# vinits5/learning3d

Hardware: AMD Instinct MI355X
Metric: clouds/sec DGCNN-fwd+Chamfer B=32 N=1024; kNN HBM GB/s vs peak at 1/2/4/8 GPU (higher is better)
Workload: dtype f32 (shared-MLP GEMMs as f16x2: fp32 operands carried as an fp16 high part + an fp16 residual (unscaled between the EdgeConv kernel and conv5, 2^12-scaled elsewhere), 3 fp16 MFMA products per fp32 product, f32 accumulate, fp32-level error -- tests bound it by 2x the fp32-MFMA kernel's own error agai

## Files before the change

### learning3d_amd/csrc/knn_mfma.hip

```cpp
#include "common.h"

typedef float f32x16 __attribute__((ext_vector_type(16)));
typedef unsigned long long u64;

#define KM_MCAP 64
#define KM_STRIDE 65
#define KM_WPAD 16
#define KM_T3S 25
#define KM_PAD (-3.0e38f)

__device__ __forceinline__ f32x16 km_tile(const float *__restrict__ cxy, const float *__restrict__ czw, int at,
                                          float b1, float b2, float b3, float a3)
{
    f32x16 acc = {0.f, 0.f, 0.f, 0.f, 0.f, 0.f, 0.f, 0.f, 0.f, 0.f, 0.f, 0.f, 0.f, 0.f, 0.f, 0.f};
    acc = __builtin_amdgcn_mfma_f32_32x32x2f32(cxy[at], b1, acc, 0, 0, 0);
    acc = __builtin_amdgcn_mfma_f32_32x32x2f32(czw[at], b2, acc, 0, 0, 0);
    acc = __builtin_amdgcn_mfma_f32_32x32x2f32(a3, b3, acc, 0, 0, 0);
    return acc;
}

__device__ __forceinline__ float km_nextup(float x)
{
    const unsigned b = __float_as_uint(x + 0.0f);
    return __uint_as_float((int)b >= 0 ? b + 1u : b - 1u);
}

#ifdef KM_TIMING
#define KMT(n) if (lane == 0) ((long long *)idx_out)[((size_t)(blockIdx.y * gridDim.x + blockIdx.x) * 4 + wave) * 16 + (n)] = __builtin_amdgcn_s_memtime();
#else
#define KMT(n)
#endif

template <int CT>
__global__ __launch_bounds__(256, 2) void knn_mfma_kernel(const float *__restrict__ xyz, int N, int k, int T_,
                                                          int64_t *__restrict__ idx_out)
{
    const int T = CT > 0 ? CT : T_;
    extern __shared__ __attribute__((aligned(16))) unsigned char km_smem[];
    const int NS = 4 * T * 32, WS = T * 32 + KM_WPAD, P = 4 * WS;
    float *cx = (float *)km_smem;
    float *cz = cx + 2 * P;
    float *dump = cx + 4 * P;
    u64 *qlist = (u64 *)(dump + 4 * 2048);
    float *t3 = (float *)(qlist + 32 * KM_STRIDE);
    float *thr0s = t3 + 32 * KM_T3S;
    int *qcnt = (int *)(thr0s + 32 * 9);
    int *ovf = qcnt + 32;

    const int tid = threadIdx.x, lane = tid & 63, wave = tid >> 6;
    const int i = lane & 31, h = lane >> 5, lane8 = 2 * wave + h;
    const int b = blockIdx.y, q0 = blockIdx.x * 32;
    const float *cloud = xyz + (size_t)b * N * 3;
    KMT(7)

    for (int c0 = tid; c0 < NS; c0 += 1024) {
        float x[4], y[4], z[4];
#pragma unroll
        for (int u = 0; u < 4; u++) {
            const int cc = min(c0 + 256 * u, N - 1);
            x[u] = cloud[cc * 3 + 0];
            y[u] = cloud[cc * 3 + 1];
            z[u] = cloud[cc * 3 + 2];
        }
#pragma unroll
        for (int u = 0; u < 4; u++)
            if (c0 + 256 * u >= N) { x[u] = 0.f; y[u] = 0.f; z[u] = 0.f; }
#pragma unroll
        for (int u = 0; u < 4; u++) {
            const int c = c0 + 256 * u;
            if (c < NS) {
                const float w = c < N ? -((x[u] * x[u] + y[u] * y[u]) + z[u] * z[u]) : KM_PAD;
                const int l8 = c & 7, s = c >> 3, j = s >> 4, r = s & 15;
                const int p = (l8 >> 1) * WS + j * 32 + ((r >> 2) << 3) + ((l8 & 1) << 2) + (r & 3);
                cx[p] = x[u];
                cx[P + p] = y[u];
                cz[p] = z[u];
                cz[P + p] = w;
            }
        }
    }
    for (int e = tid; e < 32 * KM_STRIDE; e += 256) qlist[e] = 0ull;
    if (tid < 32) qcnt[tid] = 0;
    if (tid == 0) *ovf = 0;

    const int q = q0 + i;
    const bool valid = q < N;
    const float *qp = cloud + (size_t)(valid ? q : N - 1) * 3;
    const float qx = qp[0], qy = qp[1], qz = qp[2];
    const float qxx = (qx * qx + qy * qy) + qz * qz;
    const float b1 = h ? 2.0f * qy : 2.0f * qx;
    const float b2 = h ? 1.0f : 2.0f * qz;
    const float b3 = h ? 0.0f : -qxx;
    const float a3 = h ? 0.0f : 1.0f;
    const float *cxy = cx + h * P;
    const float *czw = cz + h * P;
    const int at0 = wave * WS + i;
    KMT(0)
    __syncthreads();
    KMT(1)

    float mr[16];
#pragma unroll
    for (int r = 0; r < 16; r++) mr[r] = -INFINITY;
    f32x16 kept[CT > 0 ? CT : 1];
    int j = 0;
    if constexpr (CT > 0) {
        static_assert(CT % 2 == 0, "tiles are consumed in pairs");
#pragma unroll
        for (int t = 0; t < CT; t++) kept[t] = km_tile(cxy, czw, at0 + t * 32, b1, b2, b3, a3);
#pragma unroll
        for (int t = 0; t < CT; t += 2)
#pragma unroll
            for (int r = 0; r < 16; r++) mr[r] = fmaxf(fmaxf(mr[r], kept[t][r]), kept[t + 1][r]);
    } else {
        for (; j + 2 <= T; j += 2) {
            const f32x16 aA = km_tile(cxy, czw, at0 + j * 32, b1, b2, b3, a3);
            const f32x16 aB = km_tile(cxy, czw, at0 + j * 32 + 32, b1, b2, b3, a3);
#pragma unroll
            for (int r = 0; r < 16; r++) mr[r] = fmaxf(fmaxf(mr[r], aA[r]), aB[r]);
        }
        if (j < T) {
            const f32x16 aA = km_tile(cxy, czw, at0 + j * 32, b1, b2, b3, a3);
#pragma unroll
            for (int r = 0; r < 16; r++) mr[r] = fmaxf(mr[r], aA[r]);
        }
    }
    KMT(2)
    float m1 = -INFINITY, m2 = -INFINITY, m3 = -INFINITY;
#pragma unroll
    for (int r = 0; r < 16; r++) {
        const float v = mr[r];
        m3 = __builtin_amdgcn_fmed3f(m2, m3, v);
        m2 = __builtin_amdgcn_fmed3f(m1, m2, v);
        m1 = fmaxf(m1, v);
    }
    t3[i * KM_T3S + lane8 * 3 + 0] = m1;
    t3[i * KM_T3S + lane8 * 3 + 1] = m2;
    t3[i * KM_T3S + lane8 * 3 + 2] = m3;
    __syncthreads();
    {
        int g1 = 0, g2 = 0, g3 = 0;
#pragma unroll 8
        for (int f = 0; f < 24; f++) {
            const float v = t3[i * KM_T3S + f];
            g1 += v > m1;
            g2 += v > m2;
            g3 += v > m3;
        }
        const float offer = g3 < k ? m3 : g2 < k ? m2 : g1 < k ? m1 : INFINITY;
        thr0s[i * 9 + lane8] = offer;
    }
    __syncthreads();
    float thr0_ = thr0s[i * 9];
#pragma unroll
    for (int l = 1; l < 8; l++) thr0_ = fminf(thr0_, thr0s[i * 9 + l]);
#ifdef KM_TIMING
    float thr0 = (k & 0x100) ? INFINITY : thr0_;
    k &= 0xff;
#else
    float thr0 = thr0_;
#endif
    KMT(3)

    float *mydump = dump + wave * 2048;
    u64 *mylist = qlist + i * KM_STRIDE;
    float thr = thr0;
    bool strict = false;
    for (int attempt = 0;; attempt++) {
        const float thrc = strict ? km_nextup(thr) : thr;
        bool over = false;
    #pragma unroll
        for (j = 0; j < T; j += 2) {
            const bool two = j + 1 < T;
            f32x16 aA, aB;
            if constexpr (CT > 0) {
                aA = kept[j];
                aB = kept[j + 1];
            } else {
                aA = km_tile(cxy, czw, at0 + j * 32, b1, b2, b3, a3);
                aB = km_tile(cxy, czw, at0 + (two ? j * 32 + 32 : j * 32), b1, b2, b3, a3);
            }
            unsigned sgn = 0;
    #pragma unroll
            for (int r = 0; r < 16; r++) sgn = __builtin_amdgcn_alignbit(sgn, __float_as_uint(aA[r] - thrc), 31);
    #pragma unroll
            for (int r = 0; r < 16; r++) sgn = __builtin_amdgcn_alignbit(sgn, __float_as_uint(aB[r] - thrc), 31);
            unsigned m = ~sgn;
            if (!two) m &= 0xFFFF0000u;
            if (__builtin_amdgcn_ballot_w64(m != 0) != 0) {
    #pragma unroll
                for (int qd = 0; qd < 4; qd++) {
                    *(float4 *)(mydump + (qd * 64 + lane) * 4) = make_float4(aA[4 * qd], aA[4 * qd + 1], aA[4 * qd + 2], aA[4 * qd + 3]);
                    *(float4 *)(mydump + 1024 + (qd * 64 + lane) * 4) = make_float4(aB[4 * qd], aB[4 * qd + 1], aB[4 * qd + 2], aB[4 * qd + 3]);
                }
                const int cbase = 128 * j + lane8;
    #pragma unroll 1
                do {
                    int e[4], slot[4];
                    bool has[4];
                    float vv[4];
    #pragma unroll
                    for (int u = 0; u < 4; u++) {
                        has[u] = m != 0;
                        e[u] = has[u] ? __builtin_clz(m) : 31;
                        m &= ~(0x80000000u >> e[u]);
                        vv[u] = mydump[((e[u] >> 2) << 8) + lane * 4 + (e[u] & 3)];
                        slot[u] = atomicAdd(&qcnt[i], has[u] ? 1 : 0);
                    }
    #pragma unroll
                    for (int u = 0; u < 4; u++) {
                        const unsigned bits = __float_as_uint(vv[u] + 0.0f);
                        const unsigned sk = bits ^ ((unsigned)((int)bits >> 31) | 0x80000000u);
                        const u64 key = ((u64)sk << 32) | (unsigned)(~(cbase + 8 * e[u]));
                        const bool fits = slot[u] < KM_MCAP;
                        over |= has[u] && !fits;
                        mylist[has[u] && fits ? slot[u] : KM_MCAP] = key;
                    }
                } while (__builtin_amdgcn_ballot_w64(m != 0) != 0);
            }
        }
        if (over) *ovf = 1;
        KMT(4)
        __syncthreads();
        KMT(5)
        if (*ovf == 0) break;
        if (attempt == 64) {
            if (tid == 0) idx_out[((size_t)b * N + q0) * k] = -1;
            return;
        }
        if (lane8 == 0) thr0s[i * 9 + 8] = thr;
        __syncthreads();
        {
            u64 own[8];
            int rank[8];
#pragma unroll
            for (int o = 0; o < 8; o++) {
                own[o] = mylist[lane8 + 8 * o];
                rank[o] = 0;
            }
            for (int f = 0; f < KM_MCAP; f++) {
                const u64 kf = mylist[f];
#pragma unroll
                for (int o = 0; o < 8; o++) rank[o] += kf > own[o] ? 1 : 0;
            }
#pragma unroll
            for (int o = 0; o < 8; o++)
                if (own[o] != 0ull && rank[o] == k - 1) {
                    const unsigned sk = (unsigned)(own[o] >> 32);
                    thr0s[i * 9 + 8] = __uint_as_float((sk & 0x80000000u) ? sk ^ 0x80000000u : ~sk);
                }
        }
        __syncthreads();
        {
            const float thr_new = thr0s[i * 9 + 8];
            if (thr_new > thr) {
                thr = thr_new;
                strict = false;
            } else {
                strict = true;
            }
        }
        __syncthreads();
        for (int e = tid; e < 32 * KM_STRIDE; e += 256) qlist[e] = 0ull;
        if (tid < 32) qcnt[tid] = 0;
        if (tid == 0) *ovf = 0;
        __syncthreads();
    }

    int Mi = qcnt[i];
#pragma unroll
    for (int d = 16; d > 0; d >>= 1) Mi = max(Mi, __shfl_xor(Mi, d, 64));
    const int Mmax = __builtin_amdgcn_readfirstlane(Mi);
    u64 own[8];
    int rank[8];
#pragma unroll
    for (int o = 0; o < 8; o++) {
        own[o] = mylist[lane8 + 8 * o];
        rank[o] = 0;
    }
    if (Mmax <= 32) {
#pragma unroll 2
        for (int f = 0; f < Mmax; f++) {
            const u64 kf = mylist[f];
#pragma unroll
            for (int o = 0; o < 4; o++) rank[o] += kf > own[o] ? 1 : 0;
        }
    } else if (Mmax <= 48) {
#pragma unroll 2
        for (int f = 0; f < Mmax; f++) {
            const u64 kf = mylist[f];
#pragma unroll
            for (int o = 0; o < 6; o++) rank[o] += kf > own[o] ? 1 : 0;
        }
    } else {
#pragma unroll 2
        for (int f = 0; f < Mmax; f++) {
            const u64 kf = mylist[f];
#pragma unroll
            for (int o = 0; o < 8; o++) rank[o] += kf > own[o] ? 1 : 0;
        }
    }
    KMT(6)
#ifdef KM_TIMING
    if (lane == 0) ((long long *)idx_out)[((size_t)(blockIdx.y * gridDim.x + blockIdx.x) * 4 + wave) * 16 + 8] =
        rank[0] + rank[1] + rank[2] + rank[3] + rank[4] + rank[5] + rank[6] + rank[7];
    return;
#endif
    int64_t *dst = idx_out + ((size_t)b * N + (valid ? q : 0)) * k;
    if (valid) {
#pragma unroll
        for (int o = 0; o < 8; o++)
            if (own[o] != 0ull && rank[o] < k) dst[rank[o]] = (int64_t)(unsigned)(~(unsigned)own[o]);
    }

    const int Mq = qcnt[i];
    const int need = (strict && Mq < k) ? k - Mq : 0;
    __syncthreads();
    if (tid == 0) *ovf = 0;
    __syncthreads();
    if (need > 0) atomicMax(ovf, need);
    __syncthreads();
    const int rounds = *ovf;
    int last = -1;
    int *props = (int *)thr0s;
    for (int round = 0; round < rounds; round++) {
        int prop = 0x7fffffff;
        for (int t = T - 1; t >= 0; t--) {
            f32x16 av;
            if constexpr (CT > 0) {
                av = kept[0];
#pragma unroll
                for (int u = 1; u < CT; u++) av = t == u ? kept[u] : av;
            } else {
                av = km_tile(cxy, czw, at0 + t * 32, b1, b2, b3, a3);
            }
#pragma unroll
            for (int r = 15; r >= 0; r--) {
                const int sl = 16 * t + r;
                prop = (av[r] == thr && sl > last) ? sl : prop;
            }
        }
        const int c = prop != 0x7fffffff ? 8 * prop + lane8 : 0x7fffffff;
        props[i * 9 + lane8] = c;
        __syncthreads();
        int cmin = props[i * 9];
#pragma unroll
        for (int l = 1; l < 8; l++) cmin = min(cmin, props[i * 9 + l]);
        if (c == cmin && c != 0x7fffffff) {
            last = prop;
            if (round < need && valid) dst[Mq + round] = c;
        }
        __syncthreads();
    }
}

size_t l3d_knn_mfma_lds_bytes(int N)
{
    const int T = l3d_divup(N, 128);
    return (size_t)4 * (4 * (T * 32 + KM_WPAD)) * 4 + 4 * 2048 * 4 + 32 * KM_STRIDE * 8 + 32 * KM_T3S * 4 + 32 * 9 * 4 + 32 * 4 + 16;
}

bool l3d_knn_mfma_supported(int N, int k) { return k <= 24 && N >= 256 && N <= 2048; }

int l3d_launch_knn_mfma(const float *xyz, int B, int N, int k, int64_t *idx, hipStream_t st)
{
    const int T = l3d_divup(N, 128);
    const dim3 grid(l3d_divup(N, 32), B);
    if (T == 8)
        hipLaunchKernelGGL(knn_mfma_kernel<8>, grid, dim3(256), l3d_knn_mfma_lds_bytes(N), st, xyz, N, k, T, idx);
    else
        hipLaunchKernelGGL(knn_mfma_kernel<0>, grid, dim3(256), l3d_knn_mfma_lds_bytes(N), st, xyz, N, k, T, idx);
    return l3d_check_launch();
}
```

Measured before the change: 120,300.

## Double kNN block to 64 queries, drop kept tiles and LDS dump, recompute distances

The kNN kernel now uses 512-thread blocks that handle 64 queries with 8 waves, sharing one staged candidate set in LDS. The register-resident kept[] tiles and the per-wave LDS dump buffer are removed. Each pass recomputes tiles with a 2-MFMA product that leaves out the -|q|^2 term and subtracts it afterward, and selected candidates get their exact value recomputed from LDS coordinates with fmaf. The aim is to cut register and LDS pressure so occupancy rises and candidate loading is amortised, at the cost of redoing the MFMAs on every threshold attempt and possibly shifting tie-breaking numerics.

Result: faster. 122,800 (median of 6 runs) (+2.1%).

```diff
diff --git a/learning3d_amd/csrc/knn_mfma.hip b/learning3d_amd/csrc/knn_mfma.hip
--- a/learning3d_amd/csrc/knn_mfma.hip
+++ b/learning3d_amd/csrc/knn_mfma.hip
@@ -19,6 +19,20 @@
     return acc;
 }
 
+__device__ __forceinline__ f32x16 km_tile2(const float *__restrict__ cxy, const float *__restrict__ czw, int at, float b1, float b2)
+{
+    f32x16 acc = {0.f, 0.f, 0.f, 0.f, 0.f, 0.f, 0.f, 0.f, 0.f, 0.f, 0.f, 0.f, 0.f, 0.f, 0.f, 0.f};
+    acc = __builtin_amdgcn_mfma_f32_32x32x2f32(cxy[at], b1, acc, 0, 0, 0);
+    acc = __builtin_amdgcn_mfma_f32_32x32x2f32(czw[at], b2, acc, 0, 0, 0);
+    return acc;
+}
+
+__device__ __forceinline__ float km_value(float cx, float cy, float cz, float cw, float tqx, float tqy, float tqz, float qxx)
+{
+    const float d = fmaf(cz, tqz, fmaf(cy, tqy, cx * tqx));
+    return (d + cw) - qxx;
+}
+
 __device__ __forceinline__ float km_nextup(float x)
 {
     const unsigned b = __float_as_uint(x + 0.0f);
@@ -26,13 +40,13 @@
 }
 
 #ifdef KM_TIMING
-#define KMT(n) if (lane == 0) ((long long *)idx_out)[((size_t)(blockIdx.y * gridDim.x + blockIdx.x) * 4 + wave) * 16 + (n)] = __builtin_amdgcn_s_memtime();
+#define KMT(n) if (lane == 0) ((long long *)idx_out)[((size_t)(blockIdx.y * gridDim.x + blockIdx.x) * 8 + wave) * 16 + (n)] = __builtin_amdgcn_s_memtime();
 #else
 #define KMT(n)
 #endif
 
 template <int CT>
-__global__ __launch_bounds__(256, 2) void knn_mfma_kernel(const float *__restrict__ xyz, int N, int k, int T_,
+__global__ __launch_bounds__(512, 4) void knn_mfma_kernel(const float *__restrict__ xyz, int N, int k, int T_,
                                                           int64_t *__restrict__ idx_out)
 {
     const int T = CT > 0 ? CT : T_;
@@ -40,34 +54,34 @@
     const int NS = 4 * T * 32, WS = T * 32 + KM_WPAD, P = 4 * WS;
     float *cx = (float *)km_smem;
     float *cz = cx + 2 * P;
-    float *dump = cx + 4 * P;
-    u64 *qlist = (u64 *)(dump + 4 * 2048);
-    float *t3 = (float *)(qlist + 32 * KM_STRIDE);
-    float *thr0s = t3 + 32 * KM_T3S;
-    int *qcnt = (int *)(thr0s + 32 * 9);
-    int *ovf = qcnt + 32;
-
-    const int tid = threadIdx.x, lane = tid & 63, wave = tid >> 6;
-    const int i = lane & 31, h = lane >> 5, lane8 = 2 * wave + h;
-    const int b = blockIdx.y, q0 = blockIdx.x * 32;
+    u64 *qlist = (u64 *)(cx + 4 * P);
+    float *t3 = (float *)(qlist + 64 * KM_STRIDE);
+    float *thr0s = t3 + 64 * KM_T3S;
+    int *qcnt = (int *)(thr0s + 64 * 9);
+    int *ovf = qcnt + 64;
+
+    const int tid = threadIdx.x, lane = tid & 63, wave = tid >> 6, wq = wave & 3;
+    const int i = lane & 31, h = lane >> 5, lane8 = 2 * wq + h;
+    const int qi = (wave >> 2) * 32 + i;
+    const int b = blockIdx.y, q0 = blockIdx.x * 64;
     const float *cloud = xyz + (size_t)b * N * 3;
     KMT(7)
 
-    for (int c0 = tid; c0 < NS; c0 += 1024) {
+    for (int c0 = tid; c0 < NS; c0 += 2048) {
         float x[4], y[4], z[4];
 #pragma unroll
         for (int u = 0; u < 4; u++) {
-            const int cc = min(c0 + 256 * u, N - 1);
+            const int cc = min(c0 + 512 * u, N - 1);
             x[u] = cloud[cc * 3 + 0];
             y[u] = cloud[cc * 3 + 1];
             z[u] = cloud[cc * 3 + 2];
         }
 #pragma unroll
         for (int u = 0; u < 4; u++)
-            if (c0 + 256 * u >= N) { x[u] = 0.f; y[u] = 0.f; z[u] = 0.f; }
+            if (c0 + 512 * u >= N) { x[u] = 0.f; y[u] = 0.f; z[u] = 0.f; }
 #pragma unroll
         for (int u = 0; u < 4; u++) {
-            const int c = c0 + 256 * u;
+            const int c = c0 + 512 * u;
             if (c < NS) {
                 const float w = c < N ? -((x[u] * x[u] + y[u] * y[u]) + z[u] * z[u]) : KM_PAD;
                 const int l8 = c & 7, s = c >> 3, j = s >> 4, r = s & 15;
@@ -79,22 +93,23 @@
             }
         }
     }
-    for (int e = tid; e < 32 * KM_STRIDE; e += 256) qlist[e] = 0ull;
-    if (tid < 32) qcnt[tid] = 0;
+    for (int e = tid; e < 64 * KM_STRIDE; e += 512) qlist[e] = 0ull;
+    if (tid < 64) qcnt[tid] = 0;
     if (tid == 0) *ovf = 0;
 
-    const int q = q0 + i;
+    const int q = q0 + qi;
     const bool valid = q < N;
     const float *qp = cloud + (size_t)(valid ? q : N - 1) * 3;
     const float qx = qp[0], qy = qp[1], qz = qp[2];
     const float qxx = (qx * qx + qy * qy) + qz * qz;
-    const float b1 = h ? 2.0f * qy : 2.0f * qx;
-    const float b2 = h ? 1.0f : 2.0f * qz;
+    const float tqx = 2.0f * qx, tqy = 2.0f * qy, tqz = 2.0f * qz;
+    const float b1 = h ? tqy : tqx;
+    const float b2 = h ? 1.0f : tqz;
     const float b3 = h ? 0.0f : -qxx;
     const float a3 = h ? 0.0f : 1.0f;
     const float *cxy = cx + h * P;
     const float *czw = cz + h * P;
-    const int at0 = wave * WS + i;
+    const int at0 = wq * WS + i;
     KMT(0)
     __syncthreads();
     KMT(1)
@@ -102,29 +117,21 @@
     float mr[16];
 #pragma unroll
     for (int r = 0; r < 16; r++) mr[r] = -INFINITY;
-    f32x16 kept[CT > 0 ? CT : 1];
     int j = 0;
-    if constexpr (CT > 0) {
-        static_assert(CT % 2 == 0, "tiles are consumed in pairs");
-#pragma unroll
-        for (int t = 0; t < CT; t++) kept[t] = km_tile(cxy, czw, at0 + t * 32, b1, b2, b3, a3);
-#pragma unroll
-        for (int t = 0; t < CT; t += 2)
-#pragma unroll
-            for (int r = 0; r < 16; r++) mr[r] = fmaxf(fmaxf(mr[r], kept[t][r]), kept[t + 1][r]);
-    } else {
-        for (; j + 2 <= T; j += 2) {
-            const f32x16 aA = km_tile(cxy, czw, at0 + j * 32, b1, b2, b3, a3);
-            const f32x16 aB = km_tile(cxy, czw, at0 + j * 32 + 32, b1, b2, b3, a3);
-#pragma unroll
-            for (int r = 0; r < 16; r++) mr[r] = fmaxf(fmaxf(mr[r], aA[r]), aB[r]);
-        }
-        if (j < T) {
-            const f32x16 aA = km_tile(cxy, czw, at0 + j * 32, b1, b2, b3, a3);
-#pragma unroll
-            for (int r = 0; r < 16; r++) mr[r] = fmaxf(mr[r], aA[r]);
-        }
-    }
+    for (; j + 2 <= T; j += 2) {
+        const f32x16 aA = km_tile2(cxy, czw, at0 + j * 32, b1, b2);
+        const f32x16 aB = km_tile2(cxy, czw, at0 + j * 32 + 32, b1, b2);
+#pragma unroll
+        for (int r = 0; r < 16; r++) mr[r] = fmaxf(fmaxf(mr[r], aA[r]), aB[r]);
+        __builtin_amdgcn_sched_barrier(0);
+    }
+    if (j < T) {
+        const f32x16 aA = km_tile2(cxy, czw, at0 + j * 32, b1, b2);
+#pragma unroll
+        for (int r = 0; r < 16; r++) mr[r] = fmaxf(mr[r], aA[r]);
+    }
+#pragma unroll
+    for (int r = 0; r < 16; r++) mr[r] = (mr[r] - qxx) + 0.0f;
     KMT(2)
     float m1 = -INFINITY, m2 = -INFINITY, m3 = -INFINITY;
 #pragma unroll
@@ -134,26 +141,26 @@
         m2 = __builtin_amdgcn_fmed3f(m1, m2, v);
         m1 = fmaxf(m1, v);
     }
-    t3[i * KM_T3S + lane8 * 3 + 0] = m1;
-    t3[i * KM_T3S + lane8 * 3 + 1] = m2;
-    t3[i * KM_T3S + lane8 * 3 + 2] = m3;
+    t3[qi * KM_T3S + lane8 * 3 + 0] = m1;
+    t3[qi * KM_T3S + lane8 * 3 + 1] = m2;
+    t3[qi * KM_T3S + lane8 * 3 + 2] = m3;
     __syncthreads();
     {
         int g1 = 0, g2 = 0, g3 = 0;
 #pragma unroll 8
         for (int f = 0; f < 24; f++) {
-            const float v = t3[i * KM_T3S + f];
+            const float v = t3[qi * KM_T3S + f];
             g1 += v > m1;
             g2 += v > m2;
             g3 += v > m3;
         }
         const float offer = g3 < k ? m3 : g2 < k ? m2 : g1 < k ? m1 : INFINITY;
-        thr0s[i * 9 + lane8] = offer;
-    }
-    __syncthreads();
-    float thr0_ = thr0s[i * 9];
-#pragma unroll
-    for (int l = 1; l < 8; l++) thr0_ = fminf(thr0_, thr0s[i * 9 + l]);
+        thr0s[qi * 9 + lane8] = offer;
+    }
+    __syncthreads();
+    float thr0_ = thr0s[qi * 9];
+#pragma unroll
+    for (int l = 1; l < 8; l++) thr0_ = fminf(thr0_, thr0s[qi * 9 + l]);
 #ifdef KM_TIMING
     float thr0 = (k & 0x100) ? INFINITY : thr0_;
     k &= 0xff;
@@ -162,54 +169,60 @@
 #endif
     KMT(3)
 
-    float *mydump = dump + wave * 2048;
-    u64 *mylist = qlist + i * KM_STRIDE;
+    u64 *mylist = qlist + qi * KM_STRIDE;
+    const int pbase = wq * WS + 4 * h;
     float thr = thr0;
     bool strict = false;
     for (int attempt = 0;; attempt++) {
-        const float thrc = strict ? km_nextup(thr) : thr;
+        const float thrt = strict ? km_nextup(thr) : thr;
+        const float thrc = thrt == 0.0f ? -0.0f : thrt;
         bool over = false;
-    #pragma unroll
-        for (j = 0; j < T; j += 2) {
-            const bool two = j + 1 < T;
-            f32x16 aA, aB;
-            if constexpr (CT > 0) {
-                aA = kept[j];
-                aB = kept[j + 1];
-            } else {
-                aA = km_tile(cxy, czw, at0 + j * 32, b1, b2, b3, a3);
-                aB = km_tile(cxy, czw, at0 + (two ? j * 32 + 32 : j * 32), b1, b2, b3, a3);
-            }
-            unsigned sgn = 0;
-    #pragma unroll
-            for (int r = 0; r < 16; r++) sgn = __builtin_amdgcn_alignbit(sgn, __float_as_uint(aA[r] - thrc), 31);
-    #pragma unroll
-            for (int r = 0; r < 16; r++) sgn = __builtin_amdgcn_alignbit(sgn, __float_as_uint(aB[r] - thrc), 31);
-            unsigned m = ~sgn;
-            if (!two) m &= 0xFFFF0000u;
+    #pragma unroll 1
+        for (j = 0; j < T; j += 4) {
+            u64 m = 0;
+    #pragma unroll
+            for (int jp = 0; jp < 4; jp += 2) {
+                const int jj = j + jp;
+                unsigned mp = 0;
+                if (jj < T) {
+                    const bool two = jj + 1 < T;
+                    const f32x16 aA = km_tile2(cxy, czw, at0 + jj * 32, b1, b2);
+                    const f32x16 aB = km_tile2(cxy, czw, at0 + (two ? jj * 32 + 32 : jj * 32), b1, b2);
+                    unsigned sgn = 0;
+    #pragma unroll
+                    for (int r = 0; r < 16; r++) sgn = __builtin_amdgcn_alignbit(sgn, __float_as_uint((aA[r] - qxx) - thrc), 31);
+    #pragma unroll
+                    for (int r = 0; r < 16; r++) sgn = __builtin_amdgcn_alignbit(sgn, __float_as_uint((aB[r] - qxx) - thrc), 31);
+                    mp = ~sgn;
+                    if (!two) mp &= 0xFFFF0000u;
+                }
+                m = (m << 32) | mp;
+                __builtin_amdgcn_sched_barrier(0);
+            }
             if (__builtin_amdgcn_ballot_w64(m != 0) != 0) {
-    #pragma unroll
-                for (int qd = 0; qd < 4; qd++) {
-                    *(float4 *)(mydump + (qd * 64 + lane) * 4) = make_float4(aA[4 * qd], aA[4 * qd + 1], aA[4 * qd + 2], aA[4 * qd + 3]);
-                    *(float4 *)(mydump + 1024 + (qd * 64 + lane) * 4) = make_float4(aB[4 * qd], aB[4 * qd + 1], aB[4 * qd + 2], aB[4 * qd + 3]);
-                }
+                const int pj = pbase + 32 * j;
                 const int cbase = 128 * j + lane8;
     #pragma unroll 1
                 do {
                     int e[4], slot[4];
                     bool has[4];
-                    float vv[4];
+                    float vx[4], vy[4], vz[4], vw[4];
     #pragma unroll
                     for (int u = 0; u < 4; u++) {
                         has[u] = m != 0;
-                        e[u] = has[u] ? __builtin_clz(m) : 31;
-                        m &= ~(0x80000000u >> e[u]);
-                        vv[u] = mydump[((e[u] >> 2) << 8) + lane * 4 + (e[u] & 3)];
-                        slot[u] = atomicAdd(&qcnt[i], has[u] ? 1 : 0);
+                        e[u] = has[u] ? __builtin_clzll(m) : 63;
+                        m &= ~(0x8000000000000000ull >> e[u]);
+                        const int p = pj + e[u] + (e[u] & ~3);
+                        vx[u] = cx[p];
+                        vy[u] = cx[P + p];
+                        vz[u] = cz[p];
+                        vw[u] = cz[P + p];
+                        slot[u] = atomicAdd(&qcnt[qi], has[u] ? 1 : 0);
                     }
     #pragma unroll
                     for (int u = 0; u < 4; u++) {
-                        const unsigned bits = __float_as_uint(vv[u] + 0.0f);
+                        const float vv = km_value(vx[u], vy[u], vz[u], vw[u], tqx, tqy, tqz, qxx);
+                        const unsigned bits = __float_as_uint(vv + 0.0f);
                         const unsigned sk = bits ^ ((unsigned)((int)bits >> 31) | 0x80000000u);
                         const u64 key = ((u64)sk << 32) | (unsigned)(~(cbase + 8 * e[u]));
                         const bool fits = slot[u] < KM_MCAP;
@@ -228,7 +241,7 @@
             if (tid == 0) idx_out[((size_t)b * N + q0) * k] = -1;
             return;
         }
-        if (lane8 == 0) thr0s[i * 9 + 8] = thr;
+        if (lane8 == 0) thr0s[qi * 9 + 8] = thr;
         __syncthreads();
         {
             u64 own[8];
@@ -247,12 +260,12 @@
             for (int o = 0; o < 8; o++)
                 if (own[o] != 0ull && rank[o] == k - 1) {
                     const unsigned sk = (unsigned)(own[o] >> 32);
-                    thr0s[i * 9 + 8] = __uint_as_float((sk & 0x80000000u) ? sk ^ 0x80000000u : ~sk);
+                    thr0s[qi * 9 + 8] = __uint_as_float((sk & 0x80000000u) ? sk ^ 0x80000000u : ~sk);
                 }
         }
         __syncthreads();
         {
-            const float thr_new = thr0s[i * 9 + 8];
+            const float thr_new = thr0s[qi * 9 + 8];
             if (thr_new > thr) {
                 thr = thr_new;
                 strict = false;
@@ -261,13 +274,13 @@
             }
         }
         __syncthreads();
-        for (int e = tid; e < 32 * KM_STRIDE; e += 256) qlist[e] = 0ull;
-        if (tid < 32) qcnt[tid] = 0;
+        for (int e = tid; e < 64 * KM_STRIDE; e += 512) qlist[e] = 0ull;
+        if (tid < 64) qcnt[tid] = 0;
         if (tid == 0) *ovf = 0;
         __syncthreads();
     }
 
-    int Mi = qcnt[i];
+    int Mi = qcnt[qi];
 #pragma unroll
     for (int d = 16; d > 0; d >>= 1) Mi = max(Mi, __shfl_xor(Mi, d, 64));
     const int Mmax = __builtin_amdgcn_readfirstlane(Mi);
@@ -302,7 +315,7 @@
     }
     KMT(6)
 #ifdef KM_TIMING
-    if (lane == 0) ((long long *)idx_out)[((size_t)(blockIdx.y * gridDim.x + blockIdx.x) * 4 + wave) * 16 + 8] =
+    if (lane == 0) ((long long *)idx_out)[((size_t)(blockIdx.y * gridDim.x + blockIdx.x) * 8 + wave) * 16 + 8] =
         rank[0] + rank[1] + rank[2] + rank[3] + rank[4] + rank[5] + rank[6] + rank[7];
     return;
 #endif
@@ -313,7 +326,7 @@
             if (own[o] != 0ull && rank[o] < k) dst[rank[o]] = (int64_t)(unsigned)(~(unsigned)own[o]);
     }
 
-    const int Mq = qcnt[i];
+    const int Mq = qcnt[qi];
     const int need = (strict && Mq < k) ? k - Mq : 0;
     __syncthreads();
     if (tid == 0) *ovf = 0;
@@ -326,14 +339,7 @@
     for (int round = 0; round < rounds; round++) {
         int prop = 0x7fffffff;
         for (int t = T - 1; t >= 0; t--) {
-            f32x16 av;
-            if constexpr (CT > 0) {
-                av = kept[0];
-#pragma unroll
-                for (int u = 1; u < CT; u++) av = t == u ? kept[u] : av;
-            } else {
-                av = km_tile(cxy, czw, at0 + t * 32, b1, b2, b3, a3);
-            }
+            const f32x16 av = km_tile(cxy, czw, at0 + t * 32, b1, b2, b3, a3);
 #pragma unroll
             for (int r = 15; r >= 0; r--) {
                 const int sl = 16 * t + r;
@@ -341,11 +347,11 @@
             }
         }
         const int c = prop != 0x7fffffff ? 8 * prop + lane8 : 0x7fffffff;
-        props[i * 9 + lane8] = c;
-        __syncthreads();
-        int cmin = props[i * 9];
-#pragma unroll
-        for (int l = 1; l < 8; l++) cmin = min(cmin, props[i * 9 + l]);
+        props[qi * 9 + lane8] = c;
+        __syncthreads();
+        int cmin = props[qi * 9];
+#pragma unroll
+        for (int l = 1; l < 8; l++) cmin = min(cmin, props[qi * 9 + l]);
         if (c == cmin && c != 0x7fffffff) {
             last = prop;
             if (round < need && valid) dst[Mq + round] = c;
@@ -357,7 +363,7 @@
 size_t l3d_knn_mfma_lds_bytes(int N)
 {
     const int T = l3d_divup(N, 128);
-    return (size_t)4 * (4 * (T * 32 + KM_WPAD)) * 4 + 4 * 2048 * 4 + 32 * KM_STRIDE * 8 + 32 * KM_T3S * 4 + 32 * 9 * 4 + 32 * 4 + 16;
+    return (size_t)4 * (4 * (T * 32 + KM_WPAD)) * 4 + 64 * KM_STRIDE * 8 + 64 * KM_T3S * 4 + 64 * 9 * 4 + 64 * 4 + 16;
 }
 
 bool l3d_knn_mfma_supported(int N, int k) { return k <= 24 && N >= 256 && N <= 2048; }
@@ -365,10 +371,10 @@
 int l3d_launch_knn_mfma(const float *xyz, int B, int N, int k, int64_t *idx, hipStream_t st)
 {
     const int T = l3d_divup(N, 128);
-    const dim3 grid(l3d_divup(N, 32), B);
+    const dim3 grid(l3d_divup(N, 64), B);
     if (T == 8)
-        hipLaunchKernelGGL(knn_mfma_kernel<8>, grid, dim3(256), l3d_knn_mfma_lds_bytes(N), st, xyz, N, k, T, idx);
+        hipLaunchKernelGGL(knn_mfma_kernel<8>, grid, dim3(512), l3d_knn_mfma_lds_bytes(N), st, xyz, N, k, T, idx);
     else
-        hipLaunchKernelGGL(knn_mfma_kernel<0>, grid, dim3(256), l3d_knn_mfma_lds_bytes(N), st, xyz, N, k, T, idx);
+        hipLaunchKernelGGL(knn_mfma_kernel<0>, grid, dim3(512), l3d_knn_mfma_lds_bytes(N), st, xyz, N, k, T, idx);
     return l3d_check_launch();
 }
```
